# duwt/OrienMask

Measured on AMD Instinct MI355X. Metric: images/sec end-to-end (544^2, bs=32) forward+postprocess, higher is better.
Workload: dtype f32 (fp32 tensors and accumulation; products from hi/lo fp16 pairs of the fp32 operands, three fp16 MFMAs per product group)

## Files before the change

include/orienmask_hip.h:

```cpp
#ifndef ORIENMASK_HIP_H
#define ORIENMASK_HIP_H

#include <stddef.h>
#include <stdint.h>

#ifdef __cplusplus
extern "C" {
#endif

#define OM_VERSION 140

#define OM_OK 0
#define OM_EINVAL (-1)
#define OM_ESTATE (-2)
#define OM_ENOMEM (-3)
#define OM_EHIP (-4)

#define OM_MAX_SCALES 3
#define OM_MAX_ANCHORS 9

typedef struct om_model om_model;
typedef void* om_stream;

typedef struct om_layer_info {
// ... 107 lines not shown
                           int cout, int leaky, float* out, int out_pix_stride, int32_t* status_dev, om_stream stream);
int om_conv2d_winograd24_split(const float* in, int B, int H, int W, int cin, int in_pix_stride, const void* u_split,
                               const float* scale_split, const float* shift, int cout, int leaky, const float* res,
                               int res_pix_stride, float* out, int out_pix_stride, void* scratch, size_t scratch_bytes,
                               int32_t* status_dev, om_stream stream);
int om_conv2d_wino14_split(const float* in, int B, int H, int W, int cin, int in_pix_stride, const void* u14_split,
                           const float* scale_split, const float* shift, int cout, int leaky, const float* res,
                           int res_pix_stride, float* out, int out_pix_stride, int32_t* status_dev, om_stream stream);
size_t om_conv2d_wino14_wide_scratch_bytes(int B, int H, int W, int cin);
int om_conv2d_wino14_wide(const float* in, int B, int H, int W, int cin, int in_pix_stride, const void* u14_split,
                          const float* scale_split, const float* shift, int cout, int leaky, const float* res,
                          int res_pix_stride, float* out, int out_pix_stride, void* scratch, size_t scratch_bytes,
                          int32_t* status_dev, om_stream stream);
int om_set_wino14_wide(int on);
int om_get_wino14_wide(void);
int om_set_stem_fusion(int which, int on);
int om_get_stem_fusion(int which);
int om_set_conv3x3_f16_variant(int mode);
int om_get_conv3x3_f16_variant(void);
int om_conv2d_stem(const float* in, int B, int H, int W, const float* w, const float* scale,
                   const float* shift, int cout, float* out, om_stream stream);
int om_conv2d_stem2_split(const float* in, int B, int H, int W, const float* w1, const float* scale1, const float* shift1,
                          const void* w2_split, const float* scale2_split, const float* shift2, int cout2, int leaky2, float* out,
                          int out_pix_stride, int32_t* status_dev, om_stream stream);
int om_conv2d_stem3_split(const float* in, int B, int H, int W, const float* w1, const float* scale1, const float* shift1,
                          const void* w2_split, const float* scale2_split, const float* shift2, int cout2, int leaky2, float* out,
                          int out_pix_stride, const void* w3_split, const float* scale3_split, const float* shift3, int cout3, int leaky3,
                          float* out3, int out3_pix_stride, int32_t* status_dev, om_stream stream);
int om_conv2d_stem2_f16(const float* in, int B, int H, int W, const float* w1, const float* scale1, const float* shift1,
                        const void* w2_f16, const float* scale2, const float* shift2, int cout2, int leaky2, void* out,
// ... 206 lines not shown
```

orienmask_amd/csrc/conv_wino14.hip:

```cpp
#include "wino14_shared.h"

namespace om {

constexpr int W14_RING = 4;
constexpr int W14_EMAX = 144;
constexpr int W14_VPLANE = W14_EMAX * 4;
constexpr int W14_VBUF = 6 * W14_VPLANE;
constexpr int W14_UGRP = 3 * W14_BN * 4;
constexpr int W14_THREADS = 768;

template <int MODE>
__global__ __launch_bounds__(W14_THREADS, 3) void wino14_split_kernel(const Wino14Params p) {
    __shared__ f32x4 smem[2 * W14_VBUF + W14_RING * W14_UGRP + 1];
    int* const s_ticket = reinterpret_cast<int*>(smem + 2 * W14_VBUF + W14_RING * W14_UGRP);
    f32x4* const s_u = smem + 2 * W14_VBUF;

    const int tid = threadIdx.x;
    const int lane = tid & 63;
    const int wave = __builtin_amdgcn_readfirstlane(tid >> 6);
    const int ngroups = 6 * p.nch;

    int q_xcd = 0, q_hops = 0;
    auto draw_tile = [&]() {
        const int m_tiles = p.total_tiles / p.n_tiles;
        while (q_hops < 8) {
            const int q = (q_xcd + q_hops) & 7;
            const int pm0 = (int)((long long)m_tiles * q >> 3), pm1 = (int)((long long)m_tiles * (q + 1) >> 3);
            const int v = atomicAdd(p.ticket + q, 1);
            if (v < (pm1 - pm0) * p.n_tiles) return pm0 * p.n_tiles + v;
            ++q_hops;
        }
        return p.total_tiles;
    };
    if (tid == 512) {
        asm volatile("s_getreg_b32 %0, hwreg(HW_REG_XCC_ID)" : "=s"(q_xcd));
        q_xcd &= 7;
        s_ticket[0] = draw_tile();
    }
    asm volatile("s_waitcnt lgkmcnt(0)" ::: "memory");
    __builtin_amdgcn_s_barrier();
    int tile = __builtin_amdgcn_readfirstlane(s_ticket[0]);
    int tslot = 0;

    if (wave >= 8) {
// ... 276 lines not shown
                issue_group(ub, 1);
                issue_group(ub, 2);
            }
        });
        tl = tn;
        tile = next_tile;
        tslot ^= 1;
    }
}

constexpr int W14B_UGRP = 2 * W14_UGRP;

struct Wino14VParams {
    const float* in;
    _Float16* v;
    int B, H, W, in_ps, in_bytes, nch, TW, gtot;
    long long items;
};

__device__ __forceinline__ f32x4 w14_point(const f32x4 (&d)[6], int j) {
    const f32x4 c4 = 4.f, cm4 = -4.f, c2 = 2.f, cm2 = -2.f, cm5 = -5.f;
    switch (j) {
        case 0: return __builtin_elementwise_fma(d[2], cm5, __builtin_elementwise_fma(d[0], c4, d[4]));
        case 1: return __builtin_elementwise_fma(d[1] + d[2], cm4, d[3] + d[4]);
        case 2: return __builtin_elementwise_fma(d[1] - d[2], c4, d[4] - d[3]);
        case 3: return __builtin_elementwise_fma(d[3] - d[1], c2, d[4] - d[2]);
        case 4: return __builtin_elementwise_fma(d[3] - d[1], cm2, d[4] - d[2]);
        default: return __builtin_elementwise_fma(d[3], cm5, __builtin_elementwise_fma(d[1], c4, d[5]));
    }
}

__global__ __launch_bounds__(256) void wino14_v_kernel(const Wino14VParams p) {
    const long long id = (long long)blockIdx.x * 256 + threadIdx.x;
    if (id >= p.items) return;
    const int o = (int)(id & 1);
    long long r = id >> 1;
    const int t = (int)(r % p.TW); r /= p.TW;
    const int c = (int)(r % p.nch); r /= p.nch;
    const int b = (int)(r / p.H), y = (int)(r - (long long)b * p.H);
    const auto rs_in = __builtin_amdgcn_make_buffer_rsrc(const_cast<float*>(p.in), 0, p.in_bytes, 0x00020000);
    f32x4 d[2][6];
#pragma unroll
    for (int x = 0; x < 6; ++x) {
        const int px = 4 * t - 1 + x;
        const bool ok = (unsigned)px < (unsigned)p.W;
        const int off = ok ? (((b * p.H + y) * p.W + px) * p.in_ps + 16 * c + 8 * o) * 4 : (int)0x80000000;
        d[0][x] = __builtin_bit_cast(f32x4, __builtin_amdgcn_raw_buffer_load_b128(rs_in, off, 0, 0));
        d[1][x] = __builtin_bit_cast(f32x4, __builtin_amdgcn_raw_buffer_load_b128(rs_in, ok ? off + 16 : off, 0, 0));
    }
    const long long G = (long long)b * (p.H + 2) + y + 1;
#pragma unroll
    for (int j = 0; j < 6; ++j) {
        f16x8 h, l;
#pragma unroll
        for (int q = 0; q < 2; ++q) {
            const f32x4 v = w14_point(d[q], j);
            const f16x4 hh = __builtin_convertvector(v, f16x4);
            f32x4 rem;
#pragma unroll
            for (int k = 0; k < 4; ++k) rem[k] = __builtin_fmaf((float)hh[k], -1.0f, v[k]);
            const f16x4 ll = __builtin_convertvector(rem, f16x4);
#pragma unroll
            for (int k = 0; k < 4; ++k) { h[4 * q + k] = hh[k]; l[4 * q + k] = ll[k]; }
        }
        _Float16* e = p.v + ((((long long)c * 6 + j) * p.gtot + G) * p.TW + t) * 32;
        *reinterpret_cast<f16x8*>(e + 8 * o) = h;
        *reinterpret_cast<f16x8*>(e + 16 + 8 * o) = l;
    }
}

struct Wino14WideParams {
    Wino14Params k;
    const _Float16* v;
    int v_bytes, TW;
};

template <int MODE>
__global__ __launch_bounds__(512, 2) void wino14_wide_kernel(const Wino14WideParams pw) {
    const Wino14Params& p = pw.k;
    static_assert(W14_EMAX == 144, "the nine 1-KiB pieces of a V plane and the 128-entry sub-tile offsets below assume 144 entries");
    __shared__ f32x4 smem[2 * W14_VBUF + 2 * W14B_UGRP + 1];
    f32x4* const s_u = smem + 2 * W14_VBUF;
    int* const s_ticket = reinterpret_cast<int*>(smem + 2 * W14_VBUF + 2 * W14B_UGRP);
    const int tid = threadIdx.x, lane = tid & 63;
    const int wave = __builtin_amdgcn_readfirstlane(tid >> 6);
    const int wm2 = wave >> 2, wn4 = wave & 3;
    const int fi = lane & 31, fk = lane >> 5;
    const int ngroups = 6 * p.nch;
    const int n_tiles2 = p.n_tiles >> 1, total2 = (p.total_tiles / p.n_tiles) * n_tiles2;
    const int TW = pw.TW, hp2 = p.H + 2;
    const int ecount = (p.R + 2) * p.Ct;
    const auto rs_u = __builtin_amdgcn_make_buffer_rsrc(const_cast<_Float16*>(p.u), 0, p.u_bytes, 0x00020000);
    const auto rs_v = __builtin_amdgcn_make_buffer_rsrc(const_cast<_Float16*>(pw.v), 0, pw.v_bytes, 0x00020000);
    const int drow = lane >> 2, dcol = lane & 3;
    int dvo[3], dhalf[3];
#pragma unroll
    for (int i = 0; i < 3; ++i) {
        const int piece = wave + 8 * i;
        dhalf[i] = piece >= 12;
        const int row = 16 * (piece - 12 * dhalf[i]) + drow;
        dvo[i] = row * 64 + ((dcol ^ ((row >> 2) & 3)) * 16);
    }
    const int swB = (fi >> 2) & 3;
    const int brow = (wn4 >> 1) * (W14_UGRP) + (32 * (wn4 & 1) + fi) * 4;
// ... 16 lines not shown
            const int soff = ((t64 * p.nch + c) * 6 + w14_plane(j)) * (W14_UGRP * 16);
            __builtin_amdgcn_raw_ptr_buffer_load_lds(rs_u, (lds_ptr_t)(s_u + slot * W14B_UGRP + (wave + 8 * i) * 64), 16, dvo[i], soff, 0, 0);
        }
    };
    int vsrc[2];
    auto setup_v = [&](const Wino14Tile& tl) {
#pragma unroll
        for (int i = 0; i < 2; ++i) {
            const int e = 16 * (wave + 8 * i) + drow;
            const int rr = e / p.Ct, t = e - rr * p.Ct;
            const int sw = (e >> 2) & 3;
            const int g = tl.g0 - 1 + rr;
            const int b = g / hp2;
            const int y = g - b * hp2 - 1;
            const bool ok = e < ecount && g >= 0 && g < p.gtot && y >= 0 && y < p.H && tl.t0 + t < TW;
            vsrc[i] = ok ? ((g * TW + tl.t0 + t) * 64 + ((dcol ^ sw) * 16)) : (int)0x80000000;
        }
    };
    auto issue_v_plane = [&](int c, int pl, int vb) {
        if (c >= p.nch) return;
        const int soff = (c * 6 + pl) * (p.gtot * TW * 64);
        __builtin_amdgcn_raw_ptr_buffer_load_lds(rs_v, (lds_ptr_t)(smem + vb * W14_VBUF + pl * W14_VPLANE + wave * 64), 16, vsrc[0], soff, 0, 0);
        if (wave == 0)
            __builtin_amdgcn_raw_ptr_buffer_load_lds(rs_v, (lds_ptr_t)(smem + vb * W14_VBUF + pl * W14_VPLANE + 8 * 64), 16, vsrc[1], soff, 0, 0);
    };
    f32x16 acc[2][6];
    for (;;) {
        if (tid == 0) s_ticket[0] = atomicAdd(p.ticket + 8, 1);
        __syncthreads();
        const int tile = __builtin_amdgcn_readfirstlane(s_ticket[0]);
        __syncthreads();
        if (tile >= total2) break;
        const int tn2 = tile % n_tiles2, tm = tile / n_tiles2;
        Wino14Tile tl;
        tl.g0 = (tm / p.ncb) * p.R; tl.t0 = (tm % p.ncb) * p.Ct; tl.tile_n = 2 * tn2 + (wn4 >> 1); tl.n0 = tl.tile_n * W14_BN;
        setup_v(tl);
#pragma unroll
        for (int b = 0; b < 2; ++b)
#pragma unroll
            for (int j = 0; j < 6; ++j)
#pragma unroll
                for (int r = 0; r < 16; ++r) acc[b][j][r] = 0.f;
        issue_group(tn2, 0);
#pragma unroll
        for (int pl = 0; pl < 6; ++pl) issue_v_plane(0, pl, 0);
        asm volatile("s_waitcnt vmcnt(0)" ::: "memory");
        __builtin_amdgcn_s_barrier();
        int g = 0;
// ... 112 lines not shown
    const Wino14Shape s = wino14_shape(a, align_bytes(a.in), align_bytes(a.out), a.res != nullptr, align_bytes(a.res));
    OM_REQUIRE(s.fits(), OM_EINVAL, "wino14: %d x %d x %d: input view (%lld bytes) not 16-byte aligned, or it, the weights, %lld pixels or "
               "%lld tiles (block %d x %d) out of range", a.B, a.H, a.W, s.in_bytes, s.npix, s.total_tiles, s.R, s.Ct);
    p.in = a.in; p.u = reinterpret_cast<const _Float16*>(a.w); p.scale = a.scale; p.shift = a.shift; p.res = a.res; p.out = a.out;
    p.ticket = a.ticket; p.status = a.status;
    p.B = a.B; p.H = a.H; p.W = a.W; p.in_ps = a.in_pix_stride; p.in_bytes = (int)s.in_bytes;
    p.cout = a.cout; p.out_ps = a.out_pix_stride; p.res_ps = a.res_pix_stride; p.leaky = a.leaky;
    p.fast_io = s.fast_io ? 1 : 0;
    p.out_bytes = s.fast_io ? (int)s.out_bytes : 0;
    p.res_bytes = s.fast_io ? (int)s.res_bytes : 0;
    p.R = s.R; p.Ct = s.Ct; p.ncb = s.ncb; p.gtot = a.B * (a.H + 2);
    p.n_tiles = a.cout_pad / W14_BN;
    p.nch = a.cin / 16;
    p.total_tiles = (int)s.total_tiles;
    p.u_bytes = (int)s.u_bytes;
    return OM_OK;
}

int launch_conv_wino14_split(const ConvArgs& a, hipStream_t stream) {
    Wino14Params p;
    if (int rc = wino14_fill_params(a, p)) return rc;
    const long long total = p.total_tiles;
    const long long grid = total < 256 ? total : 256;
    if (!p.fast_io) hipLaunchKernelGGL(wino14_split_kernel<2>, dim3((unsigned)grid), dim3(W14_THREADS), 0, stream, p);
    else if (a.res) hipLaunchKernelGGL(wino14_split_kernel<1>, dim3((unsigned)grid), dim3(W14_THREADS), 0, stream, p);
    else hipLaunchKernelGGL(wino14_split_kernel<0>, dim3((unsigned)grid), dim3(W14_THREADS), 0, stream, p);
    OM_CHECK_HIP(hipGetLastError());
    return OM_OK;
}

size_t wino14_wide_scratch_floats(int B, int H, int W, int cin) {
    return (size_t)(cin / 16) * 6 * B * (H + 2) * ((W + 3) / 4) * 16;
}

bool wino14_wide_supported(const ConvArgs& a, int in_align_bytes, int out_align_bytes, bool has_res, int res_align_bytes) {
    if (!wino14_layer_kind_ok(a) || a.cout_pad % 128) return false;
    const Wino14Shape s = wino14_shape(a, in_align_bytes, out_align_bytes, has_res, res_align_bytes);
    return s.fits() && s.fast_io && wino14_wide_scratch_floats(a.B, a.H, a.W, a.cin) * 4 < 0x7FFFFFF0ull;
}

int launch_conv_wino14_wide(const ConvArgs& a, float* scratch, hipStream_t stream) {
    OM_REQUIRE(scratch && (reinterpret_cast<uintptr_t>(scratch) & 15) == 0, OM_EINVAL, "wino14 wide: scratch must be 16-byte aligned");
    OM_REQUIRE(wino14_wide_supported(a, align_bytes(a.in), align_bytes(a.out), a.res != nullptr, align_bytes(a.res)), OM_EINVAL,
               "wino14 wide: cout_pad=%d must be a multiple of 128, the views 16-byte aligned and, like V, below 2 GiB", a.cout_pad);
    Wino14WideParams pw;
    if (int rc = wino14_fill_params(a, pw.k)) return rc;
    const int TW = (a.W + 3) / 4;
    pw.TW = TW;
    pw.v = reinterpret_cast<const _Float16*>(scratch);
    pw.v_bytes = (int)(wino14_wide_scratch_floats(a.B, a.H, a.W, a.cin) * 4);
    Wino14VParams pv;
    pv.in = a.in; pv.v = reinterpret_cast<_Float16*>(scratch);
    pv.B = a.B; pv.H = a.H; pv.W = a.W; pv.in_ps = a.in_pix_stride; pv.in_bytes = pw.k.in_bytes; pv.nch = pw.k.nch; pv.TW = TW; pv.gtot = pw.k.gtot;
    pv.items = (long long)a.B * a.H * TW * pv.nch * 2;
    hipLaunchKernelGGL(wino14_v_kernel, dim3((unsigned)((pv.items + 255) / 256)), dim3(256), 0, stream, pv);
    OM_CHECK_HIP(hipGetLastError());
    if (a.mid_event) OM_CHECK_HIP(hipEventRecord(a.mid_event, stream));
    const long long total2 = (long long)(pw.k.total_tiles / pw.k.n_tiles) * (pw.k.n_tiles / 2);
    const unsigned grid = (unsigned)(total2 < 256 ? total2 : 256);
    if (a.res) hipLaunchKernelGGL(wino14_wide_kernel<1>, dim3(grid), dim3(512), 0, stream, pw);
    else hipLaunchKernelGGL(wino14_wide_kernel<0>, dim3(grid), dim3(512), 0, stream, pw);
    OM_CHECK_HIP(hipGetLastError());
    return OM_OK;
}

}
```

orienmask_amd/csrc/om_common.h:

```cpp
#pragma once
#include <hip/hip_runtime.h>
#include <cstdarg>
#include <cstdint>
#include <cstdio>

#include "../../include/orienmask_hip.h"

namespace om {

void set_error(const char* fmt, ...);

#define OM_CHECK_HIP(expr)                                                              \
    do {                                                                                \
        hipError_t _e = (expr);                                                         \
        if (_e != hipSuccess) {                                                         \
            om::set_error("%s failed: %s (%s:%d)", #expr, hipGetErrorString(_e), __FILE__, __LINE__); \
            return OM_EHIP;                                                             \
        }                                                                               \
    } while (0)

#define OM_REQUIRE(cond, code, ...)                                                     \
    do {                                                                                \
        if (!(cond)) {                                                                  \
            om::set_error(__VA_ARGS__);                                                 \
// ... 69 lines not shown
bool conv3x3_f16_supported(const ConvArgsH& a);
void conv3x3_tile_for_f16(int M, int cout_pad, int W, int kc, int* bm, int* bn);
int conv3x3_f16_get_tall();
void conv3x3_f16_set_tall(int mode);
void conv_tile_for_f16(int M, int cout_pad, int cin, int* bm, int* bn, bool gather = false);
inline size_t conv_f16_weight_halfs(int cout_pad, int ks, int cin) {
    return (size_t)cout_pad * ks * ks * cin;
}
int launch_conv_stem_f16(const float* in_nchw, int B, int H, int W, const float* w, const float* scale,
                         const float* shift, int cout, void* out_nhwc_f16, hipStream_t stream);
void conv_tile_for(int M, int cout_pad, int* bm, int* bn);
int launch_conv_winograd(const ConvArgs& a, float* scratch, hipStream_t stream);
size_t wino_scratch_floats(int B, int H, int W, int C);
int launch_conv_winograd24(const ConvArgs& a, float* scratch, hipStream_t stream);
size_t wino24_scratch_floats(int B, int H, int W, int C);
int launch_conv_wino14_split(const ConvArgs& a, hipStream_t stream);
size_t wino14_wide_scratch_floats(int B, int H, int W, int cin);
bool wino14_wide_supported(const ConvArgs& a, int in_align_bytes, int out_align_bytes, bool has_res, int res_align_bytes);
int launch_conv_wino14_wide(const ConvArgs& a, float* scratch, hipStream_t stream);
bool stem2_f16_supported(int B, int H, int W, int cout2, int out_pix_stride, int out_align_bytes);
int launch_conv_stem2_f16(const float* in_nchw, int B, int H, int W, const float* w1, const float* scale1, const float* shift1,
                          const void* w2_f16, const float* scale2, const float* shift2, int cout2, int leaky2, void* out_nhwc_f16,
                          int out_pix_stride, hipStream_t stream);
struct Stem2Third {
    const void* w_split;
    const float* scale_split;
    const float* shift;
    float* out;
    int cout, leaky, out_pix_stride;
};
bool stem2_split_supported(int B, int H, int W, int cout2, int out_pix_stride, int out_align_bytes, int cout3 = 0,
                           int out3_pix_stride = 0, int out3_align_bytes = 0);
int launch_conv_stem2_split(const float* in_nchw, int B, int H, int W, const float* w1, const float* scale1, const float* shift1,
                            const void* w2_split, const float* scale2_split, const float* shift2, int cout2, int leaky2,
// ... 12 lines not shown
```

orienmask_amd/csrc/om_model.cpp:

```cpp
#include <algorithm>
#include <atomic>
#include <cstdlib>
#include <cstring>
#include <mutex>
#include <string>
#include <vector>

#include "om_common.h"

namespace om {

static thread_local char g_err[512] = "";

void set_error(const char* fmt, ...) {
    va_list ap;
    va_start(ap, fmt);
    vsnprintf(g_err, sizeof(g_err), fmt, ap);
    va_end(ap);
}

enum : int { BUF_INPUT = -1, BUF_BBOX32 = -2, BUF_BBOX16 = -3, BUF_BBOX8 = -4, BUF_ORIENS = -5 };
constexpr int HEAD_PIX_STRIDE = 256;

struct BufDef {
// ... 25 lines not shown
    Igemm,
    Split, SplitGather, SplitDirect3x3,
    Wino, WinoFused, Wino24,
    Wino14, Wino14Wide,
    IgemmF16, IgemmF16Gather,
    Conv3x3F16, Conv3x3F16Tall,
};

struct LayerPlan {
    Form form = Form::Stem;
    int bm = 0, bn = 0;
    size_t scratch_floats = 0;
    enum Blob { F32, SPLIT, F16 } blob = F32;
    int64_t w_off = -1, scale_off = -1;
    int ksplit_max = 0;
    bool to_side = false;
    bool gather = false;
};

static int algo_code(Form f, bool f16) {
    switch (f) {
        case Form::Stem: return 0;
        case Form::Igemm: case Form::IgemmF16: return 1;
        case Form::Wino: return 2;
        case Form::WinoFused: return 3;
        case Form::Conv3x3F16: return 4;
        case Form::Wino24: case Form::IgemmF16Gather: return 5;
        case Form::Conv3x3F16Tall: return 6;
        case Form::Split: case Form::SplitDirect3x3: case Form::Stem2F16: return 7;
        case Form::Wino14: return 8;
// ... 340 lines not shown
        p.ksplit_max = latency ? latency_ksplit : 0;
        const bool wino = li.wino_planes != 0 && om::wino_enabled();
        if (wino && split) {
            int R = 0, Ct = 0, ncb = 0, nrb = 0;
            om::wino14_geometry(B, Hin, Win, &R, &Ct, &ncb, &nrb);
            const long long tiles = (long long)nrb * ncb * (li.cout_pad / 64);
            p.blob = om::LayerPlan::SPLIT;
            if (latency && tiles <= 128) {
                p.form = Form::SplitDirect3x3;
                p.w_off = li.wsplit_direct_off; p.scale_off = li.wsplit_direct_scale_off;
                om::conv_tile_for_split(B * Hin * Win, li.cout_pad, &p.bm, &p.bn);
                return p;
            }
            p.form = Form::Wino14; p.bm = 128; p.bn = 64;
            p.w_off = li.wsplit_off; p.scale_off = li.wsplit_scale_off;
            if (switch_on(SW_W14_WIDE) && li.cin >= 512 && tiles > 256 && L.in.buf >= 0 && L.out.buf >= 0 && (!L.has_res || L.res.buf >= 0)) {
                om::ConvArgs a{};
                layer_shape(a, L, p, B, H, W);
                if (om::wino14_wide_supported(a, view_align_bytes(L.in, false), view_align_bytes(L.out, false), L.has_res,
                                              L.has_res ? view_align_bytes(L.res, false) : 0)) {
                    p.form = Form::Wino14Wide; p.bn = 128;
                    p.scratch_floats = om::wino14_wide_scratch_floats(B, Hin, Win, li.cin);
                }
            }
        } else if (wino && cells >= 1700ll) {
            p.form = Form::Wino24; p.bm = 64; p.bn = 64;
            p.w_off = li.wino_off;
            p.scratch_floats = om::wino24_scratch_floats(B, Hin, Win, li.cin);
        } else if (wino) {
            const bool fused_transform = om::wino_fused_for(li.cin);
            p.form = fused_transform ? Form::WinoFused : Form::Wino;
            p.bm = 64;
            p.bn = fused_transform ? (li.cout_pad % 128 == 0 ? 128 : 64) : om::wino_bn((long long)B * ((Hin + 1) / 2) * ((Win + 1) / 2), li.cout_pad);
            p.w_off = li.wino_alt_off;
            p.scratch_floats = om::wino_scratch_floats(B, Hin, Win, li.cin);
        } else if (split && li.wino_planes == 0) {
            p.blob = om::LayerPlan::SPLIT;
            p.w_off = li.wsplit_off; p.scale_off = li.wsplit_scale_off;
            p.to_side = on_read && L.side >= 0; p.gather = on_read && !L.gather.empty();
            p.form = p.gather ? Form::SplitGather : Form::Split;
            om::conv_tile_for_split(B * Ho * Wo, li.cout_pad, &p.bm, &p.bn, p.gather);
        } else {
            p.form = Form::Igemm;
            om::conv_tile_for(B * Ho * Wo, li.cout_pad, &p.bm, &p.bn);
        }
        return p;
    }

    size_t buf_floats(int i, int B, int H, int W) const {
        return (size_t)B * (H / bufs[i].div) * (W / bufs[i].div) * bufs[i].C;
    }

    struct Layout {
        std::vector<om::LayerPlan> plans;
        std::vector<size_t> buf_off;
        std::vector<size_t> scratch_off;
        size_t tickets_off = 0, partial_off = 0, total = 0;
    };

    Layout layout(int B, int H, int W, bool f16) const {
        const size_t esz = f16 ? 2 : 4;
// ... 161 lines not shown
            const float* shift = m->weights + L.info.shift_off;
            return f16 ? om::launch_conv_stem_f16(x, B, H / L.in_div, W / L.in_div, m->weights + p.w_off, scale_of(p), shift, L.info.cout, ptr_of(L.out), stream)
                       : om::launch_conv_stem(x, B, H / L.in_div, W / L.in_div, m->weights + p.w_off, scale_of(p), shift, L.info.cout,
                                              static_cast<float*>(ptr_of(L.out)), stream);
        }
        if (f16) {
            om::ConvArgsH a = conv_args<om::ConvArgsH>(index, p);
            a.out_f32 = L.out.buf < 0 ? 1 : 0;
            if (int rc = ev.mid()) return rc;
            return om::launch_conv_igemm_f16(a, stream);
        }
        om::ConvArgs a = conv_args<om::ConvArgs>(index, p);
        a.sk_partial = sk_partial;
        a.status = status;
        a.ksplit_max = p.ksplit_max;
        a.split = p.form == Form::Wino14 || p.form == Form::Wino14Wide ? 1 : 0;
        float* scratch = reinterpret_cast<float*>(workspace + lay->scratch_off[index]);
        switch (p.form) {
            case Form::Wino: case Form::WinoFused: a.mid_event = ev.ev_mid; return om::launch_conv_winograd(a, scratch, stream);
            case Form::Wino24: a.mid_event = ev.ev_mid; return om::launch_conv_winograd24(a, scratch, stream);
            case Form::Wino14Wide: a.mid_event = ev.ev_mid; return om::launch_conv_wino14_wide(a, scratch, stream);
            default: break;
        }
        if (int rc = ev.mid()) return rc;
        switch (p.form) {
            case Form::Wino14: return om::launch_conv_wino14_split(a, stream);
            case Form::Split: case Form::SplitGather: case Form::SplitDirect3x3: return om::launch_conv_igemm_split(a, stream);
            case Form::Igemm: return om::launch_conv_igemm(a, stream);
            default: break;
        }
        om::set_error("no launch for kernel form %d", (int)p.form);
        return OM_ESTATE;
    }

    int launch_first_layers(const om::LayerPlan& p, const LayerEvents& ev) const {
        const om::LayerDef& S = m->layers[0];
        const om::LayerDef& N = m->layers[1];
        const float *w = m->weights + p.w_off, *scale = scale_of(p), *shift = m->weights + S.info.shift_off;
        const float* n_shift = m->weights + N.info.shift_off;
        const int n_stride = m->pix_stride(N.out.buf);
        if (int rc = ev.mid()) return rc;
// ... 464 lines not shown
                               int res_pix_stride, float* out, int out_pix_stride, void* scratch, size_t scratch_bytes,
                               int32_t* status_dev, om_stream stream) {
    return conv2d_winograd24_impl(in, B, H, W, cin, in_pix_stride, static_cast<const float*>(u_split), scale_split, shift, cout,
                                  leaky, res, res_pix_stride, out, out_pix_stride, scratch, scratch_bytes, stream, 1, status_dev);
}

int om_conv2d_wino14_split(const float* in, int B, int H, int W, int cin, int in_pix_stride, const void* u14_split,
                           const float* scale_split, const float* shift, int cout, int leaky, const float* res,
                           int res_pix_stride, float* out, int out_pix_stride, int32_t* status_dev, om_stream stream) {
    OM_REQUIRE(B > 0 && H > 0 && W > 0, OM_EINVAL, "om_conv2d_wino14_split: bad shape");
    om::ConvArgs a;
    a.in = in; a.w = static_cast<const float*>(u14_split); a.scale = scale_split; a.shift = shift; a.res = res; a.out = out;
    om::fill_conv_shape(a, B, H, W, cin, in_pix_stride, cout, om::round_up(cout, 64), 3, 1, leaky, res_pix_stride, out_pix_stride);
    a.split = 1; a.status = status_dev;
    if (int rc = unit_ticket(static_cast<hipStream_t>(stream), &a.ticket)) return rc;
    return om::launch_conv_wino14_split(a, static_cast<hipStream_t>(stream));
}

size_t om_conv2d_wino14_wide_scratch_bytes(int B, int H, int W, int cin) {
    if (B <= 0 || H <= 0 || W <= 0 || cin <= 0 || cin % 16) return 0;
    return om::align_up(om::wino14_wide_scratch_floats(B, H, W, cin) * sizeof(float), 256);
}

int om_conv2d_wino14_wide(const float* in, int B, int H, int W, int cin, int in_pix_stride, const void* u14_split,
                          const float* scale_split, const float* shift, int cout, int leaky, const float* res,
                          int res_pix_stride, float* out, int out_pix_stride, void* scratch, size_t scratch_bytes,
                          int32_t* status_dev, om_stream stream) {
    OM_REQUIRE(B > 0 && H > 0 && W > 0, OM_EINVAL, "om_conv2d_wino14_wide: bad shape");
    OM_REQUIRE(scratch && scratch_bytes >= om_conv2d_wino14_wide_scratch_bytes(B, H, W, cin), OM_ENOMEM,
               "om_conv2d_wino14_wide: scratch too small");
    om::ConvArgs a;
    a.in = in; a.w = static_cast<const float*>(u14_split); a.scale = scale_split; a.shift = shift; a.res = res; a.out = out;
    om::fill_conv_shape(a, B, H, W, cin, in_pix_stride, cout, om::round_up(cout, 64), 3, 1, leaky, res_pix_stride, out_pix_stride);
    a.split = 1; a.status = status_dev;
    if (int rc = unit_ticket(static_cast<hipStream_t>(stream), &a.ticket)) return rc;
    return om::launch_conv_wino14_wide(a, static_cast<float*>(scratch), static_cast<hipStream_t>(stream));
}

int om_set_wino14_wide(int on) {
    OM_REQUIRE(on == 0 || on == 1, OM_EINVAL, "om_set_wino14_wide: %d", on);
    switch_flag(SW_W14_WIDE).store(on, std::memory_order_relaxed);
    return OM_OK;
}
int om_get_wino14_wide(void) { return switch_on(SW_W14_WIDE) ? 1 : 0; }

int om_conv2d_stem3_split(const float* in, int B, int H, int W, const float* w1, const float* scale1, const float* shift1,
                          const void* w2_split, const float* scale2_split, const float* shift2, int cout2, int leaky2, float* out,
                          int out_pix_stride, const void* w3_split, const float* scale3_split, const float* shift3, int cout3, int leaky3,
                          float* out3, int out3_pix_stride, int32_t* status_dev, om_stream stream) {
    om::Stem2Third third{w3_split, scale3_split, shift3, out3, cout3, leaky3, out3_pix_stride};
    return om::launch_conv_stem2_split(in, B, H, W, w1, scale1, shift1, w2_split, scale2_split, shift2, cout2, leaky2, out,
// ... 43 lines not shown
```

orienmask_amd/csrc/wino14_shared.h:

```cpp
#pragma once
#include <cstdlib>
#include <type_traits>

#include "conv_f16_common.h"

namespace om {

typedef _Float16 f16x4 __attribute__((ext_vector_type(4)));
typedef _Float16 f16x2 __attribute__((ext_vector_type(2)));
typedef float f32x2 __attribute__((ext_vector_type(2)));
typedef unsigned u32x2 __attribute__((ext_vector_type(2)));
typedef unsigned u32x4v __attribute__((__vector_size__(4 * sizeof(unsigned))));

constexpr int W14_BM = 128, W14_BN = 64;

struct Wino14Params {
    const float* in;
    const _Float16* u;
    const float* scale;
    const float* shift;
    const float* res;
    float* out;
    int* ticket;
    int* status;
    int B, H, W, in_ps, in_bytes;
    int cout, out_ps, res_ps, leaky, fast_io, out_bytes, res_bytes;
    int R, Ct, ncb, gtot;
    int n_tiles, total_tiles, nch;
    int u_bytes;
};

__host__ __device__ constexpr int w14_plane(int g) { return g == 0 ? 0 : g == 1 ? 5 : g - 1; }

struct Wino14Tile {
    int g0, t0, n0, tile_n;
};

__device__ __forceinline__ void wino14_decode(const Wino14Params& p, int tile, Wino14Tile& t) {
    t.tile_n = tile % p.n_tiles;
    const int tm = tile / p.n_tiles;
    const int cb = tm % p.ncb, rb = tm / p.ncb;
    t.g0 = rb * p.R; t.t0 = cb * p.Ct; t.n0 = t.tile_n * W14_BN;
}

// ... 114 lines not shown
```

orienmask_amd/lib.py:

```python
import ctypes
import os

_HERE = os.path.dirname(os.path.abspath(__file__))
LIB_PATH = os.path.join(_HERE, "lib", "liborienmask_hip.so")

OM_MAX_SCALES = 3
OM_MAX_ANCHORS = 9
OM_STATUS_SPLIT_RANGE = 1
OM_STATUS_SK_TIMEOUT = 2


class LayerInfo(ctypes.Structure):
    _fields_ = [("name", ctypes.c_char * 64),
                ("cin", ctypes.c_int32), ("cout", ctypes.c_int32), ("cout_pad", ctypes.c_int32),
                ("ksize", ctypes.c_int32), ("stride", ctypes.c_int32),
                ("has_bn", ctypes.c_int32), ("leaky", ctypes.c_int32), ("wino_planes", ctypes.c_int32),
                ("w_off", ctypes.c_int64), ("scale_off", ctypes.c_int64), ("shift_off", ctypes.c_int64),
                ("wino_off", ctypes.c_int64), ("wino_alt_off", ctypes.c_int64), ("w16_off", ctypes.c_int64),
                ("wsplit_off", ctypes.c_int64), ("wsplit_scale_off", ctypes.c_int64),
                ("wsplit_direct_off", ctypes.c_int64), ("wsplit_direct_scale_off", ctypes.c_int64)]


class PostCfg(ctypes.Structure):
    _fields_ = [("num_scales", ctypes.c_int32),
# ... 77 lines not shown
    "om_model_get_precision": (_i, [_vp]),
    "om_model_set_latency_cells": (_i, [_vp, ctypes.c_longlong]),
    "om_model_set_latency_ksplit": (_i, [_vp, _i]),
    "om_model_attach_postprocess": (_i, [_vp, ctypes.POINTER(PostCfg), _vp, _vp, _vp, _vp, _vp, _vp, ctypes.c_size_t]),
    "om_model_set_upsample_on_read": (_i, [_vp, _i]),
    "om_conv2d_split": (_i, [_vp, _i, _i, _i, _i, _i, _vp, _vp, _vp, _i, _i, _i, _i, _vp, _i, _vp, _i, _i, _i, _i, _i, _vp, _vp]),
    "om_conv2d_split_k": (_i, [_vp, _i, _i, _i, _i, _i, _vp, _vp, _vp, _i, _i, _i, _i, _vp, _i, _vp, _i, _i, _i, _i, _i, _i, _vp, _vp]),
    "om_conv2d_winograd24_split": (_i, [_vp, _i, _i, _i, _i, _i, _vp, _vp, _vp, _i, _i, _vp, _i, _vp, _i, _vp, _sz, _vp, _vp]),
    "om_set_stem_fusion": (_i, [_i, _i]),
    "om_get_stem_fusion": (_i, [_i]),
    "om_get_conv3x3_f16_variant": (_i, []),
    "om_set_conv3x3_f16_variant": (_i, [_i]),
    "om_conv2d_wino14_split": (_i, [_vp, _i, _i, _i, _i, _i, _vp, _vp, _vp, _i, _i, _vp, _i, _vp, _i, _vp, _vp]),
    "om_conv2d_wino14_wide_scratch_bytes": (_sz, [_i, _i, _i, _i]),
    "om_conv2d_wino14_wide": (_i, [_vp, _i, _i, _i, _i, _i, _vp, _vp, _vp, _i, _i, _vp, _i, _vp, _i, _vp, _sz, _vp, _vp]),
    "om_set_wino14_wide": (_i, [_i]),
    "om_get_wino14_wide": (_i, []),
    "om_forward_workspace_bytes": (_sz, [_vp, _i, _i, _i]),
    "om_forward_status_offset": (_sz, [_vp, _i, _i, _i]),
    "om_forward": (_i, [_vp, _vp, _i, _i, _i, _vp, _vp, _vp, _vp, _vp, _sz, _vp]),
    "om_layer_tile": (_i, [_vp, _i, _i, _i, _i, ctypes.POINTER(ctypes.c_int), ctypes.POINTER(ctypes.c_int),
                           ctypes.POINTER(ctypes.c_int)]),
    "om_model_weight_halfs": (_sz, [_vp]),
    "om_model_load_weights_f16": (_i, [_vp, _vp, _sz]),
    "om_forward_f16_workspace_bytes": (_sz, [_vp, _i, _i, _i]),
    "om_forward_f16": (_i, [_vp, _vp, _i, _i, _i, _vp, _vp, _vp, _vp, _vp, _sz, _vp]),
    "om_layer_tile_f16": (_i, [_vp, _i, _i, _i, _i, ctypes.POINTER(ctypes.c_int), ctypes.POINTER(ctypes.c_int),
                               ctypes.POINTER(ctypes.c_int)]),
    "om_conv2d_f16": (_i, [_vp, _i, _i, _i, _i, _i, _vp, _vp, _vp, _i, _i, _i, _i, _vp, _i, _vp, _i, _i, _vp]),
    "om_conv2d_stem_f16": (_i, [_vp, _i, _i, _i, _vp, _vp, _vp, _i, _vp, _vp]),
# ... 115 lines not shown
```

Baseline: 2177.

## Split wino14 layers by M-block range between wide and split kernels

```diff
diff --git a/include/orienmask_hip.h b/include/orienmask_hip.h
--- a/include/orienmask_hip.h
+++ b/include/orienmask_hip.h
@@ -145,6 +145,12 @@
                           int32_t* status_dev, om_stream stream);
 int om_set_wino14_wide(int on);
 int om_get_wino14_wide(void);
+int om_conv2d_wino14_mblocks(int B, int H, int W);
+size_t om_conv2d_wino14_rows_scratch_bytes(int B, int H, int W, int cin, int wide_mblocks);
+int om_conv2d_wino14_rows(const float* in, int B, int H, int W, int cin, int in_pix_stride, const void* u14_split,
+                          const float* scale_split, const float* shift, int cout, int leaky, const float* res,
+                          int res_pix_stride, float* out, int out_pix_stride, int wide_mblocks, void* scratch, size_t scratch_bytes,
+                          int32_t* status_dev, om_stream stream);
 int om_set_stem_fusion(int which, int on);
 int om_get_stem_fusion(int which);
 int om_set_conv3x3_f16_variant(int mode);
diff --git a/orienmask_amd/csrc/conv_wino14.hip b/orienmask_amd/csrc/conv_wino14.hip
--- a/orienmask_amd/csrc/conv_wino14.hip
+++ b/orienmask_amd/csrc/conv_wino14.hip
@@ -22,12 +22,12 @@
 
     int q_xcd = 0, q_hops = 0;
     auto draw_tile = [&]() {
-        const int m_tiles = p.total_tiles / p.n_tiles;
+        const int m_tiles = p.mcnt;
         while (q_hops < 8) {
             const int q = (q_xcd + q_hops) & 7;
             const int pm0 = (int)((long long)m_tiles * q >> 3), pm1 = (int)((long long)m_tiles * (q + 1) >> 3);
             const int v = atomicAdd(p.ticket + q, 1);
-            if (v < (pm1 - pm0) * p.n_tiles) return pm0 * p.n_tiles + v;
+            if (v < (pm1 - pm0) * p.n_tiles) return (p.mb0 + pm0) * p.n_tiles + v;
             ++q_hops;
         }
         return p.total_tiles;
@@ -334,7 +334,9 @@
 struct Wino14VParams {
     const float* in;
     _Float16* v;
-    int B, H, W, in_ps, in_bytes, nch, TW, gtot;
+    int B, H, W, in_ps, in_bytes, nch, TW;
+    int row0;
+    int g_base, vrows;
     long long items;
 };
 
@@ -357,6 +359,7 @@
     long long r = id >> 1;
     const int t = (int)(r % p.TW); r /= p.TW;
     const int c = (int)(r % p.nch); r /= p.nch;
+    r += p.row0;
     const int b = (int)(r / p.H), y = (int)(r - (long long)b * p.H);
     const auto rs_in = __builtin_amdgcn_make_buffer_rsrc(const_cast<float*>(p.in), 0, p.in_bytes, 0x00020000);
     f32x4 d[2][6];
@@ -368,7 +371,7 @@
         d[0][x] = __builtin_bit_cast(f32x4, __builtin_amdgcn_raw_buffer_load_b128(rs_in, off, 0, 0));
         d[1][x] = __builtin_bit_cast(f32x4, __builtin_amdgcn_raw_buffer_load_b128(rs_in, ok ? off + 16 : off, 0, 0));
     }
-    const long long G = (long long)b * (p.H + 2) + y + 1;
+    const long long G = (long long)b * (p.H + 2) + y + 1 - p.g_base;
 #pragma unroll
     for (int j = 0; j < 6; ++j) {
         f16x8 h, l;
@@ -383,7 +386,7 @@
 #pragma unroll
             for (int k = 0; k < 4; ++k) { h[4 * q + k] = hh[k]; l[4 * q + k] = ll[k]; }
         }
-        _Float16* e = p.v + ((((long long)c * 6 + j) * p.gtot + G) * p.TW + t) * 32;
+        _Float16* e = p.v + ((((long long)c * 6 + j) * p.vrows + G) * p.TW + t) * 32;
         *reinterpret_cast<f16x8*>(e + 8 * o) = h;
         *reinterpret_cast<f16x8*>(e + 16 + 8 * o) = l;
     }
@@ -393,6 +396,8 @@
     Wino14Params k;
     const _Float16* v;
     int v_bytes, TW;
+    int v_row0_bytes;
+    int v_plane_bytes;
 };
 
 template <int MODE>
@@ -407,7 +412,7 @@
     const int wm2 = wave >> 2, wn4 = wave & 3;
     const int fi = lane & 31, fk = lane >> 5;
     const int ngroups = 6 * p.nch;
-    const int n_tiles2 = p.n_tiles >> 1, total2 = (p.total_tiles / p.n_tiles) * n_tiles2;
+    const int n_tiles2 = p.n_tiles >> 1, total2 = p.mcnt * n_tiles2;
     const int TW = pw.TW, hp2 = p.H + 2;
     const int ecount = (p.R + 2) * p.Ct;
     const auto rs_u = __builtin_amdgcn_make_buffer_rsrc(const_cast<_Float16*>(p.u), 0, p.u_bytes, 0x00020000);
@@ -454,12 +459,12 @@
             const int b = g / hp2;
             const int y = g - b * hp2 - 1;
             const bool ok = e < ecount && g >= 0 && g < p.gtot && y >= 0 && y < p.H && tl.t0 + t < TW;
-            vsrc[i] = ok ? ((g * TW + tl.t0 + t) * 64 + ((dcol ^ sw) * 16)) : (int)0x80000000;
+            vsrc[i] = ok ? ((g * TW + tl.t0 + t) * 64 - pw.v_row0_bytes + ((dcol ^ sw) * 16)) : (int)0x80000000;
         }
     };
     auto issue_v_plane = [&](int c, int pl, int vb) {
         if (c >= p.nch) return;
-        const int soff = (c * 6 + pl) * (p.gtot * TW * 64);
+        const int soff = (c * 6 + pl) * pw.v_plane_bytes;
         __builtin_amdgcn_raw_ptr_buffer_load_lds(rs_v, (lds_ptr_t)(smem + vb * W14_VBUF + pl * W14_VPLANE + wave * 64), 16, vsrc[0], soff, 0, 0);
         if (wave == 0)
             __builtin_amdgcn_raw_ptr_buffer_load_lds(rs_v, (lds_ptr_t)(smem + vb * W14_VBUF + pl * W14_VPLANE + 8 * 64), 16, vsrc[1], soff, 0, 0);
@@ -471,7 +476,7 @@
         const int tile = __builtin_amdgcn_readfirstlane(s_ticket[0]);
         __syncthreads();
         if (tile >= total2) break;
-        const int tn2 = tile % n_tiles2, tm = tile / n_tiles2;
+        const int tn2 = tile % n_tiles2, tm = p.mb0 + tile / n_tiles2;
         Wino14Tile tl;
         tl.g0 = (tm / p.ncb) * p.R; tl.t0 = (tm % p.ncb) * p.Ct; tl.tile_n = 2 * tn2 + (wn4 >> 1); tl.n0 = tl.tile_n * W14_BN;
         setup_v(tl);
@@ -614,14 +619,52 @@
     p.nch = a.cin / 16;
     p.total_tiles = (int)s.total_tiles;
     p.u_bytes = (int)s.u_bytes;
+    p.mb0 = 0; p.mcnt = s.nrb * s.ncb;
     return OM_OK;
 }
 
-int launch_conv_wino14_split(const ConvArgs& a, hipStream_t stream) {
+int wino14_compute_units() {
+    static const int cus = [] {
+        int dev = 0, n = 0;
+        if (hipGetDevice(&dev) != hipSuccess || hipDeviceGetAttribute(&n, hipDeviceAttributeMultiprocessorCount, dev) != hipSuccess || n < 1) {
+            (void)hipGetLastError();
+            n = 256;
+        }
+        return n;
+    }();
+    return cus;
+}
+
+int wino14_mblocks(int B, int H, int W) {
+    int R = 0, Ct = 0, ncb = 0, nrb = 0;
+    wino14_geometry(B, H, W, &R, &Ct, &ncb, &nrb);
+    return nrb * ncb;
+}
+
+static void wino14_rows_of(int B, int H, int W, int mb0, int mb1, int* g_base, int* vrows, long long* row0, long long* row1) {
+    int R = 0, Ct = 0, ncb = 0, nrb = 0;
+    wino14_geometry(B, H, W, &R, &Ct, &ncb, &nrb);
+    const long long gtot = (long long)B * (H + 2);
+    long long ga = (long long)(mb0 / ncb) * R - 1, gb = (long long)((mb1 + ncb - 1) / ncb) * R + 1;
+    if (ga < 0) ga = 0;
+    if (gb > gtot) gb = gtot;
+    auto image_rows_below = [&](long long g) {
+        const long long b = g / (H + 2), rem = g - b * (H + 2) - 1;
+        return b * H + (rem < 0 ? 0 : rem > H ? H : rem);
+    };
+    *g_base = (int)ga; *vrows = (int)(gb - ga);
+    *row0 = image_rows_below(ga); *row1 = image_rows_below(gb);
+}
+
+static bool wino14_range_ok(const ConvArgs& a, int mb0, int mb1) { return mb0 >= 0 && mb0 < mb1 && mb1 <= wino14_mblocks(a.B, a.H, a.W); }
+
+int launch_conv_wino14_split(const ConvArgs& a, int mb0, int mb1, hipStream_t stream) {
     Wino14Params p;
     if (int rc = wino14_fill_params(a, p)) return rc;
-    const long long total = p.total_tiles;
-    const long long grid = total < 256 ? total : 256;
+    OM_REQUIRE(wino14_range_ok(a, mb0, mb1), OM_EINVAL, "wino14: M blocks [%d, %d) of %d", mb0, mb1, p.total_tiles / p.n_tiles);
+    p.mb0 = mb0; p.mcnt = mb1 - mb0;
+    const long long total = (long long)p.mcnt * p.n_tiles, cus = wino14_compute_units();
+    const long long grid = total < cus ? total : cus;
     if (!p.fast_io) hipLaunchKernelGGL(wino14_split_kernel<2>, dim3((unsigned)grid), dim3(W14_THREADS), 0, stream, p);
     else if (a.res) hipLaunchKernelGGL(wino14_split_kernel<1>, dim3((unsigned)grid), dim3(W14_THREADS), 0, stream, p);
     else hipLaunchKernelGGL(wino14_split_kernel<0>, dim3((unsigned)grid), dim3(W14_THREADS), 0, stream, p);
@@ -629,9 +672,13 @@
     return OM_OK;
 }
 
-size_t wino14_wide_scratch_floats(int B, int H, int W, int cin) {
-    return (size_t)(cin / 16) * 6 * B * (H + 2) * ((W + 3) / 4) * 16;
-}
+size_t wino14_wide_scratch_floats(int B, int H, int W, int cin, int mb0, int mb1) {
+    int g_base = 0, vrows = 0;
+    long long row0 = 0, row1 = 0;
+    wino14_rows_of(B, H, W, mb0, mb1, &g_base, &vrows, &row0, &row1);
+    return (size_t)(cin / 16) * 6 * vrows * ((W + 3) / 4) * 16;
+}
+size_t wino14_wide_scratch_floats(int B, int H, int W, int cin) { return wino14_wide_scratch_floats(B, H, W, cin, 0, wino14_mblocks(B, H, W)); }
 
 bool wino14_wide_supported(const ConvArgs& a, int in_align_bytes, int out_align_bytes, bool has_res, int res_align_bytes) {
     if (!wino14_layer_kind_ok(a) || a.cout_pad % 128) return false;
@@ -639,25 +686,32 @@
     return s.fits() && s.fast_io && wino14_wide_scratch_floats(a.B, a.H, a.W, a.cin) * 4 < 0x7FFFFFF0ull;
 }
 
-int launch_conv_wino14_wide(const ConvArgs& a, float* scratch, hipStream_t stream) {
+int launch_conv_wino14_wide(const ConvArgs& a, float* scratch, int mb0, int mb1, hipStream_t stream) {
     OM_REQUIRE(scratch && (reinterpret_cast<uintptr_t>(scratch) & 15) == 0, OM_EINVAL, "wino14 wide: scratch must be 16-byte aligned");
     OM_REQUIRE(wino14_wide_supported(a, align_bytes(a.in), align_bytes(a.out), a.res != nullptr, align_bytes(a.res)), OM_EINVAL,
                "wino14 wide: cout_pad=%d must be a multiple of 128, the views 16-byte aligned and, like V, below 2 GiB", a.cout_pad);
     Wino14WideParams pw;
     if (int rc = wino14_fill_params(a, pw.k)) return rc;
+    OM_REQUIRE(wino14_range_ok(a, mb0, mb1), OM_EINVAL, "wino14 wide: M blocks [%d, %d) of %d", mb0, mb1, pw.k.total_tiles / pw.k.n_tiles);
+    pw.k.mb0 = mb0; pw.k.mcnt = mb1 - mb0;
     const int TW = (a.W + 3) / 4;
+    long long row0 = 0, row1 = 0;
+    int g_base = 0, vrows = 0;
+    wino14_rows_of(a.B, a.H, a.W, mb0, mb1, &g_base, &vrows, &row0, &row1);
+    pw.v_row0_bytes = g_base * TW * 64; pw.v_plane_bytes = vrows * TW * 64;
     pw.TW = TW;
     pw.v = reinterpret_cast<const _Float16*>(scratch);
-    pw.v_bytes = (int)(wino14_wide_scratch_floats(a.B, a.H, a.W, a.cin) * 4);
+    pw.v_bytes = (int)(wino14_wide_scratch_floats(a.B, a.H, a.W, a.cin, mb0, mb1) * 4);
     Wino14VParams pv;
     pv.in = a.in; pv.v = reinterpret_cast<_Float16*>(scratch);
-    pv.B = a.B; pv.H = a.H; pv.W = a.W; pv.in_ps = a.in_pix_stride; pv.in_bytes = pw.k.in_bytes; pv.nch = pw.k.nch; pv.TW = TW; pv.gtot = pw.k.gtot;
-    pv.items = (long long)a.B * a.H * TW * pv.nch * 2;
-    hipLaunchKernelGGL(wino14_v_kernel, dim3((unsigned)((pv.items + 255) / 256)), dim3(256), 0, stream, pv);
+    pv.B = a.B; pv.H = a.H; pv.W = a.W; pv.in_ps = a.in_pix_stride; pv.in_bytes = pw.k.in_bytes; pv.nch = pw.k.nch; pv.TW = TW;
+    pv.row0 = (int)row0; pv.g_base = g_base; pv.vrows = vrows;
+    pv.items = (row1 - row0) * TW * pv.nch * 2;
+    if (pv.items > 0) hipLaunchKernelGGL(wino14_v_kernel, dim3((unsigned)((pv.items + 255) / 256)), dim3(256), 0, stream, pv);
     OM_CHECK_HIP(hipGetLastError());
     if (a.mid_event) OM_CHECK_HIP(hipEventRecord(a.mid_event, stream));
-    const long long total2 = (long long)(pw.k.total_tiles / pw.k.n_tiles) * (pw.k.n_tiles / 2);
-    const unsigned grid = (unsigned)(total2 < 256 ? total2 : 256);
+    const long long total2 = (long long)pw.k.mcnt * (pw.k.n_tiles / 2), cus = wino14_compute_units();
+    const unsigned grid = (unsigned)(total2 < cus ? total2 : cus);
     if (a.res) hipLaunchKernelGGL(wino14_wide_kernel<1>, dim3(grid), dim3(512), 0, stream, pw);
     else hipLaunchKernelGGL(wino14_wide_kernel<0>, dim3(grid), dim3(512), 0, stream, pw);
     OM_CHECK_HIP(hipGetLastError());
diff --git a/orienmask_amd/csrc/om_common.h b/orienmask_amd/csrc/om_common.h
--- a/orienmask_amd/csrc/om_common.h
+++ b/orienmask_amd/csrc/om_common.h
@@ -107,10 +107,13 @@
 size_t wino_scratch_floats(int B, int H, int W, int C);
 int launch_conv_winograd24(const ConvArgs& a, float* scratch, hipStream_t stream);
 size_t wino24_scratch_floats(int B, int H, int W, int C);
-int launch_conv_wino14_split(const ConvArgs& a, hipStream_t stream);
+int wino14_mblocks(int B, int H, int W);
+int wino14_compute_units();
+int launch_conv_wino14_split(const ConvArgs& a, int mb0, int mb1, hipStream_t stream);
 size_t wino14_wide_scratch_floats(int B, int H, int W, int cin);
+size_t wino14_wide_scratch_floats(int B, int H, int W, int cin, int mb0, int mb1);
 bool wino14_wide_supported(const ConvArgs& a, int in_align_bytes, int out_align_bytes, bool has_res, int res_align_bytes);
-int launch_conv_wino14_wide(const ConvArgs& a, float* scratch, hipStream_t stream);
+int launch_conv_wino14_wide(const ConvArgs& a, float* scratch, int mb0, int mb1, hipStream_t stream);
 bool stem2_f16_supported(int B, int H, int W, int cout2, int out_pix_stride, int out_align_bytes);
 int launch_conv_stem2_f16(const float* in_nchw, int B, int H, int W, const float* w1, const float* scale1, const float* shift1,
                           const void* w2_f16, const float* scale2, const float* shift2, int cout2, int leaky2, void* out_nhwc_f16,
diff --git a/orienmask_amd/csrc/om_model.cpp b/orienmask_amd/csrc/om_model.cpp
--- a/orienmask_amd/csrc/om_model.cpp
+++ b/orienmask_amd/csrc/om_model.cpp
@@ -63,6 +63,7 @@
     enum Blob { F32, SPLIT, F16 } blob = F32;
     int64_t w_off = -1, scale_off = -1;
     int ksplit_max = 0;
+    int mblocks = 0, wide_mblocks = 0;
     bool to_side = false;
     bool gather = false;
 };
@@ -433,14 +434,15 @@
             }
             p.form = Form::Wino14; p.bm = 128; p.bn = 64;
             p.w_off = li.wsplit_off; p.scale_off = li.wsplit_scale_off;
-            if (switch_on(SW_W14_WIDE) && li.cin >= 512 && tiles > 256 && L.in.buf >= 0 && L.out.buf >= 0 && (!L.has_res || L.res.buf >= 0)) {
+            p.mblocks = nrb * ncb;
+            if (switch_on(SW_W14_WIDE) && L.in.buf >= 0 && L.out.buf >= 0 && (!L.has_res || L.res.buf >= 0)) {
                 om::ConvArgs a{};
                 layer_shape(a, L, p, B, H, W);
                 if (om::wino14_wide_supported(a, view_align_bytes(L.in, false), view_align_bytes(L.out, false), L.has_res,
-                                              L.has_res ? view_align_bytes(L.res, false) : 0)) {
-                    p.form = Form::Wino14Wide; p.bn = 128;
-                    p.scratch_floats = om::wino14_wide_scratch_floats(B, Hin, Win, li.cin);
-                }
+                                              L.has_res ? view_align_bytes(L.res, false) : 0))
+                    p.wide_mblocks = wide_blocks(li.cin, p.mblocks, li.cout_pad / 64);
+                if (p.wide_mblocks > 0) p.scratch_floats = om::wino14_wide_scratch_floats(B, Hin, Win, li.cin, 0, p.wide_mblocks);
+                if (2 * p.wide_mblocks > p.mblocks) { p.form = Form::Wino14Wide; p.bn = 128; }
             }
         } else if (wino && cells >= 1700ll) {
             p.form = Form::Wino24; p.bm = 64; p.bn = 64;
@@ -464,6 +466,10 @@
             om::conv_tile_for(B * Ho * Wo, li.cout_pad, &p.bm, &p.bn);
         }
         return p;
+    }
+
+    static int wide_blocks(int cin, int mblocks, int n_tiles) {
+        return cin >= 512 && (long long)mblocks * n_tiles > om::wino14_compute_units() ? mblocks : 0;
     }
 
     size_t buf_floats(int i, int B, int H, int W) const {
@@ -655,17 +661,23 @@
         a.sk_partial = sk_partial;
         a.status = status;
         a.ksplit_max = p.ksplit_max;
-        a.split = p.form == Form::Wino14 || p.form == Form::Wino14Wide ? 1 : 0;
+        const bool w14 = p.form == Form::Wino14 || p.form == Form::Wino14Wide;
+        a.split = w14 ? 1 : 0;
         float* scratch = reinterpret_cast<float*>(workspace + lay->scratch_off[index]);
         switch (p.form) {
             case Form::Wino: case Form::WinoFused: a.mid_event = ev.ev_mid; return om::launch_conv_winograd(a, scratch, stream);
             case Form::Wino24: a.mid_event = ev.ev_mid; return om::launch_conv_winograd24(a, scratch, stream);
-            case Form::Wino14Wide: a.mid_event = ev.ev_mid; return om::launch_conv_wino14_wide(a, scratch, stream);
             default: break;
+        }
+        if (w14) {
+            if (p.wide_mblocks > 0) {
+                a.mid_event = ev.ev_mid;
+                if (int rc = om::launch_conv_wino14_wide(a, scratch, 0, p.wide_mblocks, stream)) return rc;
+            } else if (int rc = ev.mid()) return rc;
+            return p.wide_mblocks < p.mblocks ? om::launch_conv_wino14_split(a, p.wide_mblocks, p.mblocks, stream) : OM_OK;
         }
         if (int rc = ev.mid()) return rc;
         switch (p.form) {
-            case Form::Wino14: return om::launch_conv_wino14_split(a, stream);
             case Form::Split: case Form::SplitGather: case Form::SplitDirect3x3: return om::launch_conv_igemm_split(a, stream);
             case Form::Igemm: return om::launch_conv_igemm(a, stream);
             default: break;
@@ -1160,7 +1172,7 @@
     om::fill_conv_shape(a, B, H, W, cin, in_pix_stride, cout, om::round_up(cout, 64), 3, 1, leaky, res_pix_stride, out_pix_stride);
     a.split = 1; a.status = status_dev;
     if (int rc = unit_ticket(static_cast<hipStream_t>(stream), &a.ticket)) return rc;
-    return om::launch_conv_wino14_split(a, static_cast<hipStream_t>(stream));
+    return om::launch_conv_wino14_split(a, 0, om::wino14_mblocks(B, H, W), static_cast<hipStream_t>(stream));
 }
 
 size_t om_conv2d_wino14_wide_scratch_bytes(int B, int H, int W, int cin) {
@@ -1180,7 +1192,36 @@
     om::fill_conv_shape(a, B, H, W, cin, in_pix_stride, cout, om::round_up(cout, 64), 3, 1, leaky, res_pix_stride, out_pix_stride);
     a.split = 1; a.status = status_dev;
     if (int rc = unit_ticket(static_cast<hipStream_t>(stream), &a.ticket)) return rc;
-    return om::launch_conv_wino14_wide(a, static_cast<float*>(scratch), static_cast<hipStream_t>(stream));
+    return om::launch_conv_wino14_wide(a, static_cast<float*>(scratch), 0, om::wino14_mblocks(B, H, W), static_cast<hipStream_t>(stream));
+}
+
+int om_conv2d_wino14_mblocks(int B, int H, int W) {
+    if (B <= 0 || H <= 0 || W <= 0) return 0;
+    return om::wino14_mblocks(B, H, W);
+}
+
+size_t om_conv2d_wino14_rows_scratch_bytes(int B, int H, int W, int cin, int wide_mblocks) {
+    if (B <= 0 || H <= 0 || W <= 0 || cin <= 0 || cin % 16 || wide_mblocks <= 0 || wide_mblocks > om::wino14_mblocks(B, H, W)) return 0;
+    return om::align_up(om::wino14_wide_scratch_floats(B, H, W, cin, 0, wide_mblocks) * sizeof(float), 256);
+}
+
+int om_conv2d_wino14_rows(const float* in, int B, int H, int W, int cin, int in_pix_stride, const void* u14_split,
+                          const float* scale_split, const float* shift, int cout, int leaky, const float* res,
+                          int res_pix_stride, float* out, int out_pix_stride, int wide_mblocks, void* scratch, size_t scratch_bytes,
+                          int32_t* status_dev, om_stream stream) {
+    OM_REQUIRE(B > 0 && H > 0 && W > 0 && cin > 0 && cin % 16 == 0, OM_EINVAL, "om_conv2d_wino14_rows: bad shape");
+    const int all = om::wino14_mblocks(B, H, W);
+    OM_REQUIRE(wide_mblocks >= 0 && wide_mblocks <= all, OM_EINVAL, "om_conv2d_wino14_rows: %d wide M blocks of %d", wide_mblocks, all);
+    OM_REQUIRE(wide_mblocks == 0 || (scratch && scratch_bytes >= om_conv2d_wino14_rows_scratch_bytes(B, H, W, cin, wide_mblocks)), OM_ENOMEM,
+               "om_conv2d_wino14_rows: scratch too small for %d wide M blocks", wide_mblocks);
+    om::ConvArgs a;
+    a.in = in; a.w = static_cast<const float*>(u14_split); a.scale = scale_split; a.shift = shift; a.res = res; a.out = out;
+    om::fill_conv_shape(a, B, H, W, cin, in_pix_stride, cout, om::round_up(cout, 64), 3, 1, leaky, res_pix_stride, out_pix_stride);
+    a.split = 1; a.status = status_dev;
+    if (int rc = unit_ticket(static_cast<hipStream_t>(stream), &a.ticket)) return rc;
+    if (wide_mblocks > 0)
+        if (int rc = om::launch_conv_wino14_wide(a, static_cast<float*>(scratch), 0, wide_mblocks, static_cast<hipStream_t>(stream))) return rc;
+    return wide_mblocks < all ? om::launch_conv_wino14_split(a, wide_mblocks, all, static_cast<hipStream_t>(stream)) : OM_OK;
 }
 
 int om_set_wino14_wide(int on) {
diff --git a/orienmask_amd/csrc/wino14_shared.h b/orienmask_amd/csrc/wino14_shared.h
--- a/orienmask_amd/csrc/wino14_shared.h
+++ b/orienmask_amd/csrc/wino14_shared.h
@@ -28,6 +28,7 @@
     int R, Ct, ncb, gtot;
     int n_tiles, total_tiles, nch;
     int u_bytes;
+    int mb0, mcnt;
 };
 
 __host__ __device__ constexpr int w14_plane(int g) { return g == 0 ? 0 : g == 1 ? 5 : g - 1; }
diff --git a/orienmask_amd/lib.py b/orienmask_amd/lib.py
--- a/orienmask_amd/lib.py
+++ b/orienmask_amd/lib.py
@@ -115,6 +115,9 @@
     "om_conv2d_wino14_split": (_i, [_vp, _i, _i, _i, _i, _i, _vp, _vp, _vp, _i, _i, _vp, _i, _vp, _i, _vp, _vp]),
     "om_conv2d_wino14_wide_scratch_bytes": (_sz, [_i, _i, _i, _i]),
     "om_conv2d_wino14_wide": (_i, [_vp, _i, _i, _i, _i, _i, _vp, _vp, _vp, _i, _i, _vp, _i, _vp, _i, _vp, _sz, _vp, _vp]),
+    "om_conv2d_wino14_mblocks": (_i, [_i, _i, _i]),
+    "om_conv2d_wino14_rows_scratch_bytes": (_sz, [_i, _i, _i, _i, _i]),
+    "om_conv2d_wino14_rows": (_i, [_vp, _i, _i, _i, _i, _i, _vp, _vp, _vp, _i, _i, _vp, _i, _vp, _i, _i, _vp, _sz, _vp, _vp]),
     "om_set_wino14_wide": (_i, [_i]),
     "om_get_wino14_wide": (_i, []),
     "om_forward_workspace_bytes": (_sz, [_vp, _i, _i, _i]),
```

New measurement: 2171. Within noise of the previous version (-0.2%).
